# alipbcs/ZetaRay

Hardware: NVIDIA H100
Metric: Mpaths/s (1spp ReSTIR PT, 1080p) (higher is better)
Workload: dtype f32

## Files before the change

### zetaray_b200/csrc/rdi.cu

```cuda
#include "zr_pixel.cuh"
#include "zr_planes.h"
#include "zr_schedule.h"

#include "zr_rdi.cuh"

namespace zr
{
namespace
{
#ifndef ZR_RDI_THREADS
#define ZR_RDI_THREADS 512
#endif
    template<uint32_t MF>
    __global__ void ZR_LB(ZR_RDI_THREADS) k_di_temporal(SceneDev sc, FrameView f, DIParams prm, zr_rdi_reservoir* __restrict__ resCurr,
        const zr_rdi_reservoir* __restrict__ resPrev, uint2* __restrict__ target, float4* __restrict__ finalImg, uint32_t dispX, uint32_t dispY,
        const uint32_t* __restrict__ order)
    {
        using SD = BSDF::ShadingDataT<MF>;
        const zr_frame_constants& fc = f.fc;
        uint2 sg = make_uint2(0, 0);
        const uint32_t groupFlat = order[blockIdx.x] * (ZR_RDI_THREADS / 64) + (threadIdx.x >> 6);
        const uint32_t tInGroup = threadIdx.x & 63;
        uint2 px = make_uint2(0xffffffffu, 0xffffffffu);
        if (groupFlat < dispX * dispY)
            px = SwizzleThreadGroup(groupFlat, 0, tInGroup & 7, tInGroup >> 3, 8, 8, dispX, 16, 4, 16 * dispY, sg);
        const long long t0 = clock64();
        bool act = !(px.x >= f.W || px.y >= f.H || px.y < prm.rowBegin || px.y >= prm.rowEnd);
        const uint32_t x = px.x, y = px.y;
        const size_t idx = act ? (size_t)y * f.W + x : 0;
        if (act)
        {
            const GFlags flags = FlagsAt(f.core, f.W, x, y);
            if (flags.invalid)
            {
                finalImg[idx] = f4(0, 0, 0, 0);
                act = false;
// ... 5 lines not shown
            }
        }
        PixelT<SD> p;
        p.surface = SD::InitEmpty();
        p.pos = f3(0); p.normal = f3(0); p.roughness = 0;
        RNG rng_thread; rng_thread.State = 0;
        int numBsdfSamples = 0;
        if (act)
        {
            p = LoadPixel<SD>(f, sc, f.core, f.coat, x, y, false, x, y);
            rng_thread = RNG::Init(x, y, fc.FrameNum);
            numBsdfSamples = (!p.surface.GlossSpecular() && p.roughness < 0.3f) ? 2 : 1;
        }
        RNG rng_group = RNG::Init(groupFlat % dispX, groupFlat / dispX, fc.FrameNum);
        const uint32_t sampleSetIdx = rng_group.UniformUintBounded_Faster(sc.numSampleSets);
        Reservoir r = RIS_InitialCandidates_Sync(act, sc, p.pos, p.normal, p.roughness, p.surface, sampleSetIdx, numBsdfSamples, rng_thread);
        if (prm.temporal)
        {
            float2 motionVec = f2(0, 0);
            TemporalCandidateT<SD> tc; tc.valid = false; tc.px = tc.py = 0; tc.pos = tc.normal = f3(0);
            tc.surface = SD::InitEmpty();
            ZR_PHASE();
            if (act)
            {
                motionVec = unpack_snorm16x2(__ldg(&f.me[idx].x));
                const float2 currUV = f2((float)x + 0.5f, (float)y + 0.5f) / f2((float)f.W, (float)f.H);
                const float2 prevUV = currUV - motionVec;
                tc = FindTemporalCandidate(f, sc, p.pos, p.normal, p.roughness, p.surface, prevUV);
            }
            TemporalResample1_Sync(act && tc.valid, sc, p.pos, p.normal, p.surface, tc, resPrev, f.W, r, rng_thread);
            if (act && prm.spatial)
// ... 6 lines not shown
        }
        AccountCost(prm.costMap, f.W, f.H, px.x, px.y, t0);
        if (!act)
            return;
        if (prm.temporal || prm.reset)
        {
            zr_rdi_reservoir rec;
            r.Write(rec, prm.M_max);
            StoreRdi(&resCurr[idx], rec);
        }
        if (!prm.spatial || !prm.temporal)
            WriteFinal(fc, finalImg, idx, r.target * r.W);
    }

    template<uint32_t MF>
    __global__ void ZR_LB(ZR_RDI_THREADS) k_di_spatial(SceneDev sc, FrameView f, DIParams prm, const zr_rdi_reservoir* __restrict__ resCurr,
        const uint2* __restrict__ target, float4* __restrict__ finalImg, uint32_t dispX, uint32_t dispY,
        const uint32_t* __restrict__ order)
    {
        using SD = BSDF::ShadingDataT<MF>;
        const zr_frame_constants& fc = f.fc;
        uint2 sg = make_uint2(0, 0);
        const uint32_t groupFlat = order[blockIdx.x] * (ZR_RDI_THREADS / 64) + (threadIdx.x >> 6);
        const uint32_t tInGroup = threadIdx.x & 63;
        uint2 px = make_uint2(0xffffffffu, 0xffffffffu);
        if (groupFlat < dispX * dispY)
            px = SwizzleThreadGroup(groupFlat, 0, tInGroup & 7, tInGroup >> 3, 8, 8, dispX, 16, 4, 16 * dispY, sg);
        const long long t0 = clock64();
        bool active = px.x < f.W && px.y < f.H && px.y >= prm.rowBegin && px.y < prm.rowEnd;
        const int x = (int)px.x, y = (int)px.y;
        const size_t idx = active ? (size_t)y * f.W + x : 0;
        if (active)
        {
            const GFlags flags = FlagsAt(f.core, f.W, x, y);
            if (flags.invalid) active = false;
            else if (flags.emissive)
            {
                WriteEmissive(fc, f, finalImg, idx);
// ... 115 lines not shown
    } sz;
    int currTemporalIdx = 0;
    bool isTemporalReservoirValid = false;
    bool resetTemporalTextures = true;
    bool patternLoaded = false;
    zr_direct_params params = Defaults();
    zr::LightingStrip strip{ "zr_direct_pass" };

    static zr_direct_params Defaults()
    {
        zr_direct_params p{};
        p.temporal_resample = 1; p.spatial_resample = 1; p.stochastic_spatial = 1; p.extra_disocclusion_sampling = 1;
        p.M_max = 20; p.alpha_min = 0.05f * 0.05f;
        return p;
    }
    zr_status Setup() { return ZR_OK; }
    zr_status OnWindowResized(uint32_t w, uint32_t h)
    {
        const size_t n = (size_t)w * h;
        Sized next;
        for (int i = 0; i < 2; i++) ZR_TRY(next.planes.Alloc(next.d_res[i], n));
        ZR_TRY(next.planes.Alloc(next.d_target, n));
        ZR_TRY(next.planes.Alloc(next.d_final, n));
        ZR_TRY(next.planes.Clear());
        sz = std::move(next);
        width = w; height = h;
        strip.ForgetSize();
        ResetFlags();
        return ZR_OK;
    }
    void ResetFlags() { currTemporalIdx = 0; isTemporalReservoirValid = false; resetTemporalTextures = true; }
// ... 20 lines not shown
        zr_status st = LightingFrame("zr_direct_pass", in, width, height, f);
        if (st != ZR_OK) return st;
        st = LoadPattern();
        if (st != ZR_OK) return st;
        const bool doTemporal = isTemporalReservoirValid && params.temporal_resample;
        const bool doSpatial = doTemporal && params.spatial_resample;
        if (doTemporal && (!in->prev.d_core || !in->prev.d_coat))
        {
            set_error("zr_direct_pass_render: temporal reuse needs the previous G-buffer");
            return ZR_ERR_INVALID_ARG;
        }
        DIParams prm{ doTemporal, doSpatial, params.stochastic_spatial, params.extra_disocclusion_sampling, params.M_max,
            params.alpha_min, resetTemporalTextures, strip.rowBegin, strip.ClampedRowEnd(height), strip.d_costMap };
        const uint32_t dispX = (width + 7) / 8, dispY = (height + 7) / 8;
        const int cur = currTemporalIdx;
        st = strip.Schedule(width, height, 8, 8, ZR_RDI_THREADS / 64);
        if (st != ZR_OK) return st;
        const BlockSchedule& sched = strip.sched;
        const bool plain = (in->scene->materialFeatures & BSDF::MF_ALL) == 0;
        ZR_PROF("k_di_temporal", stream);
        (plain ? k_di_temporal<BSDF::MF_NONE> : k_di_temporal<BSDF::MF_ALL>)<<<sched.count, ZR_RDI_THREADS, 0, stream>>>(in->scene->dev, f, prm, sz.d_res[cur], sz.d_res[1 - cur], sz.d_target, sz.d_final, dispX, dispY, sched.d_order);
        ZR_LAUNCH_CHECK();
        strip.Exchange(sz.d_res[cur], width, height, 32u, stream);
        if (doSpatial)
        {
            ZR_PROF("k_di_spatial", stream);
            (plain ? k_di_spatial<BSDF::MF_NONE> : k_di_spatial<BSDF::MF_ALL>)<<<sched.count, ZR_RDI_THREADS, 0, stream>>>(in->scene->dev, f, prm, sz.d_res[cur], sz.d_target, sz.d_final, dispX, dispY, sched.d_order);
            ZR_LAUNCH_CHECK();
        }
        isTemporalReservoirValid = true;
        currTemporalIdx = 1 - cur;
        resetTemporalTextures = false;
        return ZR_OK;
    }
};

extern "C"
{
    zr_status zr_direct_pass_create(uint32_t width, uint32_t height, zr_direct_pass** out) { return zr::CreatePass("zr_direct_pass", width, height, out); }
    zr_status zr_direct_pass_resize(zr_direct_pass* p, uint32_t width, uint32_t height) { return zr::ResizePass("zr_direct_pass", p, width, height); }
    zr_status zr_direct_pass_reset_temporal(zr_direct_pass* p) { return zr::ResetPass(p); }
    zr_status zr_direct_pass_default_params(zr_direct_params* out) { return zr::DefaultParams<zr_direct_pass>(out); }
// ... 46 lines not shown
```

### zetaray_b200/csrc/rgi.cu

```cuda
#define ZR_NO_DEGENERATE_RAY_EARLY_OUT
#include "zr_pixel.cuh"
#include "zr_rpt.cuh"
#include "zr_planes.h"
#include "zr_schedule.h"

#include "zr_rgi.cuh"

namespace zr
{
namespace
{
#ifndef ZR_RGI_THREADS
#define ZR_RGI_THREADS 1024
#endif
    template<bool PlainPT>
    __global__ void ZR_LB(ZR_RGI_THREADS) k_rgi(SceneDev sc, FrameView f, GIParams prm, zr_rgi_reservoir* __restrict__ resCurr,
        const zr_rgi_reservoir* __restrict__ resPrev, float4* __restrict__ finalImg, uint32_t dispX, uint32_t dispY,
        const uint32_t* __restrict__ order)
    {
        const zr_frame_constants& fc = f.fc;
        uint2 sg = make_uint2(0, 0);
        const uint32_t groupFlat = order[blockIdx.x] * (ZR_RGI_THREADS / 64) + (threadIdx.x >> 6);
        const uint32_t tInGroup = threadIdx.x & 63;
        uint2 px = make_uint2(0xffffffffu, 0xffffffffu);
// ... 278 lines not shown
        {
            set_error("zr_gi_pass_render: the light voxel grid is enabled but zr_build_light_voxel_grid has not run");
            return ZR_ERR_NOT_INITIALIZED;
        }
        const bool doTemporal = !plainPathTracer && params.temporal_resample && isTemporalReservoirValid;
        if (doTemporal && !in->prev.d_core)
        {
            set_error("zr_gi_pass_render: temporal reuse needs the previous G-buffer");
            return ZR_ERR_INVALID_ARG;
        }
        GIParams prm{ params.max_non_tr_bounces, params.max_glossy_tr_bounces, params.russian_roulette, params.stochastic_multi_bounce,
            params.boiling_suppression, params.M_max, doTemporal ? 1u : 0u, resetTemporalTextures ? 1u : 0u, strip.rowBegin, strip.ClampedRowEnd(height) };
        const uint32_t dispX = (width + 7) / 8, dispY = (height + 7) / 8;
        st = strip.Schedule(width, height, 8, 8, ZR_RGI_THREADS / 64);
        if (st != ZR_OK) return st;
        const BlockSchedule& sched = strip.sched;
        const int cur = currTemporalIdx;
        if (plainPathTracer)
        {
            ZR_PROF("k_pathtracer", stream);
            k_rgi<true><<<sched.count, ZR_RGI_THREADS, 0, stream>>>(in->scene->dev, f, prm, sz.d_res[cur], sz.d_res[1 - cur], sz.d_final, dispX, dispY, sched.d_order);
            ZR_LAUNCH_CHECK();
            return ZR_OK;
        }
        ZR_PROF("k_rgi", stream);
        k_rgi<false><<<sched.count, ZR_RGI_THREADS, 0, stream>>>(in->scene->dev, f, prm, sz.d_res[cur], sz.d_res[1 - cur], sz.d_final, dispX, dispY, sched.d_order);
        ZR_LAUNCH_CHECK();
        strip.Exchange(sz.d_res[cur], width, height, (uint32_t)sizeof(zr_rgi_reservoir), stream);
        isTemporalReservoirValid = true;
        currTemporalIdx = 1 - cur;
        resetTemporalTextures = false;
// ... 57 lines not shown
```

### zetaray_b200/csrc/rpt.cu

```cuda
#include "zr_rpt_io.cuh"
#include "zr_rpt_spatial.h"
#include "zr_schedule.h"

namespace zr
{
namespace
{
    using namespace RPT;

    __device__ __align__(8) float c_disk512[1024];

#ifndef ZR_PT_THREADS
#define ZR_PT_THREADS 768
#endif
    struct PtParked
    {
        Reservoir r;
        Reconnection rc;
        uint32_t pad;
    };
    static_assert(sizeof(PtParked) % 4 == 0 && (sizeof(PtParked) / 4) % 2 == 1, "PtParked must be an odd number of words");
    constexpr size_t PT_SMEM_BYTES = (size_t)ZR_PT_THREADS * sizeof(PtParked);

    template<uint32_t MF>
// ... 459 lines not shown
    zr_indirect_params params = Defaults();

    static zr_indirect_params Defaults()
    {
        zr_indirect_params p{};
        p.max_non_tr_bounces = 3; p.max_glossy_tr_bounces = 4; p.russian_roulette = 1; p.temporal_resample = 1;
        p.num_spatial_passes = 1; p.M_max_temporal = 10; p.M_max_spatial = 8; p.boiling_suppression = 1;
        p.sort_temporal = 1; p.sort_spatial = 1; p.alpha_min = 0.175f * 0.175f;
        return p;
    }

    zr_status Setup()
    {
        decltype(&zr::k_pathtrace<zr::BSDF::MF_ALL>) const kernels[2] = { zr::k_pathtrace<zr::BSDF::MF_NONE>, zr::k_pathtrace<zr::BSDF::MF_ALL> };
        for (const auto kernel : kernels)
        {
            ZR_CUDA(cudaFuncSetAttribute(kernel, cudaFuncAttributeMaxDynamicSharedMemorySize, (int)zr::PT_SMEM_BYTES));
            int ptBlocks = 0;
            ZR_CUDA(cudaOccupancyMaxActiveBlocksPerMultiprocessor(&ptBlocks, kernel, ZR_PT_THREADS, zr::PT_SMEM_BYTES));
            if (ptBlocks < 1)
            {
                zr::set_error("zr_indirect_pass: k_pathtrace (%d threads, %zu B shared) cannot be resident", ZR_PT_THREADS, zr::PT_SMEM_BYTES);
                return ZR_ERR_UNSUPPORTED;
            }
            const size_t ptSmem = (size_t)ptBlocks * (zr::PT_SMEM_BYTES + 1024);
            ZR_CUDA(cudaFuncSetAttribute(kernel, cudaFuncAttributePreferredSharedMemoryCarveout,
                (int)((ptSmem * 100 + 228 * 1024 - 1) / (228 * 1024))));
        }
        return shiftStreams.Init();
    }

    zr_status OnWindowResized(uint32_t w, uint32_t h)
    {
        const size_t n = (size_t)w * h;
        Sized next;
        for (int i = 0; i < 2; i++) ZR_TRY(next.planes.Alloc(next.d_res[i], n));
        ZR_TRY(next.planes.Alloc(next.d_threadMap, n));
        ZR_TRY(next.planes.Alloc(next.d_target, n));
        ZR_TRY(next.planes.Alloc(next.d_final, n));
        ZR_TRY(next.planes.Alloc(next.d_neighbor, n));
        ZR_TRY(next.queued.Build(w, h, next.d_res[0], next.d_res[1]));
        ZR_TRY(next.planes.Clear());
        sz = std::move(next);
// ... 41 lines not shown
        RptParams prm;
        prm.maxNonTrBounces = params.max_non_tr_bounces; prm.maxGlossyTrBounces = params.max_glossy_tr_bounces;
        prm.russianRoulette = params.russian_roulette; prm.M_max_temporal = params.M_max_temporal; prm.M_max_spatial = params.M_max_spatial;
        prm.boilingSuppression = params.boiling_suppression; prm.sortSpatial = params.sort_spatial; prm.alpha_min = params.alpha_min;
        prm.temporalResample = doTemporal; prm.resetTemporal = resetTemporalTextures; prm.spatialFlag = doSpatial;
        prm.rowBegin = strip.rowBegin; prm.rowEnd = strip.ClampedRowEnd(height);
        prm.costMap = strip.d_costMap;
        st = strip.Schedule(width, height, 16, 8, ZR_PT_THREADS / 128);
        if (st != ZR_OK) return st;
        const uint32_t rows = prm.rowEnd - prm.rowBegin;

        int cur = currTemporalIdx;
        const uint32_t dispX = (width + 15) / 16, dispY = (height + 7) / 8;
        const bool plain = (in->scene->materialFeatures & BSDF::MF_ALL) == 0;
        ZR_PROF("k_pathtrace", stream);
        (plain ? k_pathtrace<BSDF::MF_NONE> : k_pathtrace<BSDF::MF_ALL>)<<<strip.sched.count, ZR_PT_THREADS, PT_SMEM_BYTES, stream>>>(in->scene->dev, f, prm, sz.d_res[cur], sz.d_target, sz.d_final, dispX, dispY,
            strip.sched.d_order);
        ZR_LAUNCH_CHECK();
        if (doTemporal)
        {
            st = sz.queued.RunTemporal(shiftStreams, in->scene->dev, f, prm, sz.d_res[cur], sz.d_res[1 - cur], sz.d_target, sz.d_final, plain, stream);
            if (st != ZR_OK) return st;
        }
        strip.Exchange(sz.d_res[cur], width, height, 64u, stream);
        if (doSpatial)
        {
            for (uint32_t pass = 0; pass < params.num_spatial_passes; pass++)
            {
                ZR_PROF("k_spatial_search", stream);
                k_spatial_search<<<dim3((width + 31) / 32, (rows + 7) / 8), 256, 0, stream>>>(f, prm, sz.d_neighbor);
                ZR_LAUNCH_CHECK();
                zr_rpt_reservoir* rin = sz.d_res[cur];
// ... 82 lines not shown
```

### zetaray_b200/csrc/rpt_spatial.cu

```cuda
#include "zr_rpt_spatial.h"
#include "zr_rpt_shift.cuh"
#include "zr_tma.cuh"

namespace zr
{
namespace
{
    using namespace RPT;

    __global__ void __launch_bounds__(256) k_spatial_classify(FrameView f, RptParams prm, const zr_rpt_reservoir* __restrict__ resIn,
        const uint16_t* __restrict__ neighbor, uint32_t* __restrict__ queue, uint32_t* __restrict__ counters, uint32_t capacity)
    {
        __shared__ uint32_t s_count[SpatialQueued::NUM_CLASSES], s_base[SpatialQueued::NUM_CLASSES];
        const uint32_t x = blockIdx.x * 32 + (threadIdx.x & 31);
        const uint32_t y = prm.rowBegin + blockIdx.y * 8 + (threadIdx.x >> 5);
        if (threadIdx.x < SpatialQueued::NUM_CLASSES) s_count[threadIdx.x] = 0;
        __syncthreads();
        uint32_t cls[2] = { NO_ITEM, NO_ITEM };
        if (x < f.W && y < f.H && y < prm.rowEnd)
        {
            const GFlags flags = FlagsAt(f.core, f.W, (int)x, (int)y);
            int nx = 0, ny = 0;
            if (!(flags.invalid || flags.emissive) && NeighborOf(f, neighbor, (int)x, (int)y, nx, ny))
            {
// ... 252 lines not shown
                        CopyToNextFrame(rec, &resOut[idx], r_curr, M_max);
                    WriteOutputColor(fc, finalImg, idx, r_curr.target * r_curr.W);
                }
            }
            __syncthreads();
        }
    }
}

zr_status ShiftStreams::Init()
{
    int dev = 0;
    ZR_CUDA(cudaGetDevice(&dev));
    ZR_CUDA(cudaDeviceGetAttribute(&numSMs, cudaDevAttrMultiProcessorCount, dev));
    ZR_CUDA(cudaFuncSetAttribute(k_spatial_merge, cudaFuncAttributeMaxDynamicSharedMemorySize, (int)sizeof(MergeSmem)));
    for (int i = 0; i < 2; i++)
    {
        ZR_CUDA(cudaStreamCreateWithFlags(&aux[i], cudaStreamNonBlocking));
        ZR_CUDA(cudaEventCreateWithFlags(&evJoin[i], cudaEventDisableTiming));
    }
    ZR_CUDA(cudaEventCreateWithFlags(&evFork, cudaEventDisableTiming));
    return ZR_OK;
}

ShiftStreams::~ShiftStreams()
{
    for (int i = 0; i < 2; i++)
    {
        if (aux[i]) cudaStreamDestroy(aux[i]);
        if (evJoin[i]) cudaEventDestroy(evJoin[i]);
// ... 74 lines not shown
```

### zetaray_b200/csrc/rpt_temporal.cu

```cuda
#include "zr_rpt_spatial.h"
#include "zr_rpt_shift.cuh"

namespace zr
{
namespace
{
    using namespace RPT;
    enum : uint8_t { TF_OK = 1, TF_REPLAY_OK = 2 };

    __global__ void __launch_bounds__(256) k_temporal_classify(SceneDev sc, FrameView f, RptParams prm, const zr_rpt_reservoir* __restrict__ resCurr,
        const zr_rpt_reservoir* __restrict__ resPrev, uint8_t* __restrict__ tflags, uint32_t* __restrict__ queue, uint32_t* __restrict__ counters,
        uint32_t capacity)
    {
        __shared__ uint32_t s_count[SpatialQueued::NUM_CLASSES], s_base[SpatialQueued::NUM_CLASSES];
        const int x = (int)(blockIdx.x * 32 + (threadIdx.x & 31));
        const int y = (int)(prm.rowBegin + blockIdx.y * 8 + (threadIdx.x >> 5));
        if (threadIdx.x < SpatialQueued::NUM_CLASSES) s_count[threadIdx.x] = 0;
        __syncthreads();
        uint32_t cls[2] = { NO_ITEM, NO_ITEM };
        uint32_t flagBits = 0;
        if (x < (int)f.W && y < (int)f.H && y < (int)prm.rowEnd)
        {
            const size_t idx = (size_t)y * f.W + x;
            const GFlags flags = DecodeFlags(ld128(&f.core[idx]).w & 0xff);
// ... 132 lines not shown
            {
                r_curr.target = Math::Sanitize(r_curr.target);
                target[idx] = f4(r_curr.target.x, r_curr.target.y, r_curr.target.z, 0.0f);
            }
        }
        else
        {
            r_curr.WriteReservoirData(rec, M_max);
            st128(&resCurr[idx], make_uint4(rec.meta, asuint(rec.w_sum), asuint(rec.W), rec.L_b));
        }
        if (!prm.spatialFlag)
            WriteOutputColor(fc, finalImg, idx, r_curr.target * r_curr.W);
    }
}

zr_status SpatialQueued::RunTemporal(const ShiftStreams& ss, const SceneDev& sc, const FrameView& f, const RptParams& prm, zr_rpt_reservoir* resCurr,
    const zr_rpt_reservoir* resPrev, float4* target, float4* finalImg, bool plain, cudaStream_t stream)
{
    const uint32_t rows = prm.rowEnd - prm.rowBegin;
    const dim3 grid((width + 31) / 32, (rows + 7) / 8);
    ZR_CUDA(cudaMemsetAsync(d_counters, 0, 16 * sizeof(uint32_t), stream));
    {
        ZR_PROF("k_temporal_classify", stream);
        k_temporal_classify<<<grid, 256, 0, stream>>>(sc, f, prm, resCurr, resPrev, d_flags, d_queue, d_counters, (uint32_t)capacity);
        ZR_LAUNCH_CHECK();
    }
    {
        ZR_PROF("k_shift_temporal", stream);
        const zr_status ls = LaunchShifts<true>(*this, ss, sc, f, prm, resCurr, resPrev, nullptr, plain, stream);
        zr::prof_after();
// ... 13 lines not shown
```

### zetaray_b200/csrc/zr_common.cuh

```cuda
#pragma once
#include <cuda_runtime.h>
#include <stdint.h>
#include "../../include/zr_abi.h"
#include "../../include/zr_fpmath.h"

#define ZR_D __device__ __forceinline__
#ifndef ZR_MAXREGS
#define ZR_MAXREGS 0
#endif
#if ZR_MAXREGS > 0
#define ZR_LB(threads) __launch_bounds__(threads, 65536 / ((threads) * ZR_MAXREGS))
#else
#define ZR_LB(threads) __launch_bounds__(threads)
#endif

namespace zr
{
constexpr float PI = 3.141592654f;
constexpr float TWO_PI = 6.283185307f;
constexpr float PI_OVER_2 = 1.570796327f;
constexpr float PI_OVER_4 = 0.7853981635f;
constexpr float ONE_OVER_PI = 0.318309886f;
constexpr float ONE_OVER_2_PI = 0.159154943f;
constexpr float FLT_MAX_ = 3.402823466e+38f;
constexpr float FLT16_MAX = 65504.0f;

void set_error(const char* fmt, ...);
zr_status read_asset(const char* who, const char* name, void* dst, size_t bytes);
zr_status cuda_fail(cudaError_t e, const char* what);
zr_status check_frame_size(const char* pass, const zr_frame_constants& frame, uint32_t width, uint32_t height);
void count_launch(uint64_t n = 1);
#define ZR_CUDA(expr) do { cudaError_t e__ = (expr); if (e__ != cudaSuccess) return zr::cuda_fail(e__, #expr); } while (0)
#define ZR_CLEAR_BEGIN() ZR_CUDA(cudaDeviceSynchronize())
#define ZR_CLEAR_END() ZR_CUDA(cudaStreamSynchronize(cudaStreamLegacy))
void prof_before(const char* name, cudaStream_t stream);
void prof_after();
#define ZR_PROF(name, stream) zr::prof_before(name, (cudaStream_t)(stream))
#define ZR_LAUNCH_CHECK() do { zr::count_launch(); zr::prof_after(); cudaError_t e__ = cudaGetLastError(); if (e__ != cudaSuccess) return zr::cuda_fail(e__, "kernel launch"); } while (0)

ZR_D float3 f3(float x, float y, float z) { return make_float3(x, y, z); }
ZR_D float3 f3(float s) { return make_float3(s, s, s); }
ZR_D float2 f2(float x, float y) { return make_float2(x, y); }
ZR_D float4 f4(float x, float y, float z, float w) { return make_float4(x, y, z, w); }

ZR_D float3 operator+(float3 a, float3 b) { return f3(a.x + b.x, a.y + b.y, a.z + b.z); }
ZR_D float3 operator-(float3 a, float3 b) { return f3(a.x - b.x, a.y - b.y, a.z - b.z); }
ZR_D float3 operator*(float3 a, float3 b) { return f3(a.x * b.x, a.y * b.y, a.z * b.z); }
ZR_D float3 operator/(float3 a, float3 b) { return f3(a.x / b.x, a.y / b.y, a.z / b.z); }
ZR_D float3 operator*(float3 a, float s) { return f3(a.x * s, a.y * s, a.z * s); }
// ... 447 lines not shown
```

### zetaray_b200/csrc/zr_rdi.cuh

```cuda
#pragma once
#include "zr_pixel.cuh"

namespace zr
{
namespace
{
    struct DIParams
    {
        uint32_t temporal, spatial, stochasticSpatial, extraDisocclusion, M_max; float alpha_min; uint32_t reset;
        uint32_t rowBegin, rowEnd;
        unsigned long long* costMap;
    };

    __constant__ float c_disk32[64];

struct Reservoir
{
    float w_sum, W; float3 le; uint32_t lightIdx; float2 bary; uint32_t M;
    float3 target; uint32_t lightID; float3 lightPos, lightNormal; bool doubleSided;

    static ZR_D Reservoir Init()
    {
        Reservoir r;
        r.le = f3(0); r.M = 0; r.w_sum = 0; r.W = 0; r.lightIdx = UINT32_MAX_; r.bary = f2(0, 0);
// ... 99 lines not shown
    {
        wi = lightPos - pos;
        t = dot(wi, wi) == 0 ? 0 : length(wi);
        wi = t == 0 ? f3(0) : wi / t;
        lightNormal = doubleSided && dot(-wi, lightNormal) < 0 ? -lightNormal : lightNormal;
    }
    ZR_D float dWdA() const
    {
        float cosThetaPrime = saturate(dot(lightNormal, -wi));
        return t == 0 ? 0 : cosThetaPrime / (t * t);
    }
};

#define ZR_PHASE() __syncthreads()
template<class SD>
ZR_D Reservoir RIS_InitialCandidates_Sync(bool act, const SceneDev& sc, float3 pos, float3 normal, float roughness, SD surface,
    uint32_t sampleSetIdx, int numBsdfSamples, RNG& rng)
{
    Reservoir r = Reservoir::Init();
    const bool specular = surface.GlossSpecular() && (surface.metallic || surface.specTr) && (!surface.Coated() || surface.CoatSpecular());
    const int numLightSamples = !specular ? 3 : 0;
    for (int s_b = 0; s_b < 2; s_b++)
    {
        const bool go = act && (s_b < numBsdfSamples);
        BSDF::BSDFSample bsdfSample = BSDF::BSDFSample::Init();
        ZR_PHASE();
        if (go)
            bsdfSample = BSDF::SampleBSDF_NoDiffuse(normal, surface, rng);
        ZR_PHASE();
        BSDFHitInfo hitInfo;
        hitInfo.hit = false;
        if (go)
            hitInfo = FindClosestHitDI(sc, pos, normal, bsdfSample.wi, surface.Transmissive());
        ZR_PHASE();
// ... 70 lines not shown
            target *= Visibility_Segment(sc, pos, wi, t, normal, lightID, surface.Transmissive()) ? 1.0f : 0.0f;
        ZR_PHASE();
        if (go)
        {
            const float denom = (float)numLightSamples * pdf_light + (float)numBsdfSamples * BSDF::BSDFSamplerPdf_NoDiffuse(normal, surface, wi) * dwdA;
            const float m_l = denom > 0 ? 1.0f / denom : 0;
            const float w_l = m_l * Math::Luminance(target);
            if (r.Update(w_l, le, emissiveIdx, lightSample.bary, rng))
            {
                r.target = target; r.lightID = lightID; r.lightNormal = lightSample.normal; r.lightPos = lightSample.pos; r.doubleSided = doubleSided;
            }
        }
    }
    float targetLum = Math::Luminance(r.target);
    r.W = targetLum > 0.0f ? r.w_sum / targetLum : 0.0f;
    return r;
}

ZR_D bool PlaneHeuristicDI(float3 samplePos, float3 currNormal, float3 currPos, float linearDepth, float tolerance = 1e-1f)
{
    float planeDist = dot(currNormal, samplePos - currPos);
    return fabsf(planeDist) <= tolerance * linearDepth;
}

template<class SD>
struct TemporalCandidateT { SD surface; float3 pos, normal; int px, py; bool valid; };
using TemporalCandidate = TemporalCandidateT<BSDF::ShadingData>;

template<class SD>
ZR_D TemporalCandidateT<SD> FindTemporalCandidate(const FrameView& f, const SceneDev& sc, float3 pos, float3 normal, float roughness, const SD& surface, float2 prevUV)
// ... 241 lines not shown
```

### zetaray_b200/csrc/zr_rpt_shift.cuh

```cuda
#pragma once
#include "zr_rpt_spatial.h"

namespace zr
{
namespace
{
    using namespace RPT;
#ifndef ZR_SHIFT_THREADS
#define ZR_SHIFT_THREADS 512
#endif
#ifndef ZR_SHIFT_MINBLOCKS
#define ZR_SHIFT_MINBLOCKS 1
#endif
    constexpr int SHIFT_THREADS = ZR_SHIFT_THREADS, SHIFT_MINBLOCKS = ZR_SHIFT_MINBLOCKS;
    constexpr uint32_t NO_ITEM = 0xffffffffu;

    ZR_D uint32_t ShiftClass(uint32_t meta)
    {
        const uint32_t kMin2 = meta & 0xf;
        const uint32_t lt_k = (meta >> 14) & 3, lt_k1 = (meta >> 16) & 3;
        const uint32_t c = lt_k1 != 0 ? 1u : (lt_k != 0 ? 2u : 0u);
        return c * 2 + (kMin2 > 0 ? 1u : 0u);
    }


    template<int CASE, bool REPLAY, bool TEMPORAL, uint32_t MF>
    __global__ void __launch_bounds__(SHIFT_THREADS, SHIFT_MINBLOCKS) k_shift(SceneDev sc, FrameView f, RptParams prm,
        const zr_rpt_reservoir* __restrict__ resIn, const zr_rpt_reservoir* __restrict__ resPrev, const uint16_t* __restrict__ neighbor,
        const uint32_t* __restrict__ queue, uint32_t* __restrict__ counters, uint32_t cls, ShiftResult* __restrict__ out)
    {
        using SD = BSDF::ShadingDataT<MF>;
        __shared__ uint32_t s_base;
        const uint32_t total = counters[cls];
        for (;;)
        {
            __syncthreads();
            if (threadIdx.x == 0) s_base = atomicAdd(&counters[8 + cls], (uint32_t)SHIFT_THREADS);
            __syncthreads();
            const uint32_t base = s_base;
            if (base >= total) break;
            const bool act = base + threadIdx.x < total;
            int x = 0, y = 0;
            uint32_t dir = 0;
            bool replayOk = act;
            Reservoir r = Reservoir::Init();
            PixelT<SD> p, pr;
            if (act)
            {
                const uint32_t item = __ldg(&queue[base + threadIdx.x]);
                x = (int)(item & 0xffff); y = (int)((item >> 16) & 0x3fff); dir = item >> 31;
                zr_rpt_reservoir rec;
                if (!TEMPORAL)
                {
                    int nx = 0, ny = 0;
                    NeighborOf(f, neighbor, x, y, nx, ny);
                    LoadRecord(dir == 0 ? &resIn[(size_t)y * f.W + x] : &resIn[(size_t)ny * f.W + nx], rec);
                    r = Reservoir::Load_NonReconnection(rec);
                    r.rc.x_k_in_motion = false;
                    r.Load_Reconnection(rec);
                    if (dir == 0) p = LoadPixel<SD>(f, sc, f.core, f.coat, nx, ny, false, x, y);
                    else p = LoadPixel<SD>(f, sc, f.core, f.coat, x, y, false, x, y);
                    if (REPLAY)
                    {
                        if (dir == 0) pr = LoadPixel<SD>(f, sc, f.core, f.coat, nx, ny, false, nx, ny);
                        else pr = p;
                    }
                }
                else
                {
                    replayOk = ((item >> 30) & 1) != 0;
                    int ppx = 0, ppy = 0;
                    PrevPixel(f, x, y, ppx, ppy);
                    LoadRecord(dir == 0 ? &resIn[(size_t)y * f.W + x] : &resPrev[(size_t)ppy * f.W + ppx], rec);
                    r = Reservoir::Load_NonReconnection(rec);
                    r.Load_Reconnection(rec);
                    if (r.rc.IsCase1() || r.rc.IsCase2())
                    {
                        if (dir == 0) XkToPrev(sc, r.rc);
                        else XkToCurr(sc, r.rc);
                    }
                    if (dir == 0) p = LoadPixel<SD>(f, sc, f.pcore, f.pcoat, ppx, ppy, true, x, y);
                    else p = LoadPixel<SD>(f, sc, f.core, f.coat, x, y, false, x, y);
                    if (REPLAY) pr = p;
                }
            }
            OffsetPathContextT<SD> ctx = OffsetPathContextT<SD>::Init();
            if (REPLAY)
            {
                ZR_PHASE();
                ctx = Replay_kGt2_Sync(act && replayOk, sc, pr.pos, pr.normal, pr.eta_next, pr.surface, r.rc, prm.alpha_min);
                if (act && replayOk)
                    ctx = ctx.Quantize();
            }
            const OffsetPath shift = Shift2_Sync<CASE>(act, sc, p.pos, p.normal, p.eta_next, p.surface, r.rc, &ctx, prm.alpha_min);
            if (act)
            {
                ShiftResult* o = &out[(size_t)y * f.W + x];
                if (dir == 0)
                    *reinterpret_cast<float2*>(&o->ctsTargetLum) = f2(Math::Luminance(shift.target), shift.partialJacobian);
                else if (TEMPORAL)
                    st128(o, make_uint4(asuint(shift.target.x), asuint(shift.target.y), asuint(shift.target.z), asuint(shift.partialJacobian)));
                else
                {
                    const float J = shift.partialJacobian;
                    const float Jenc = J > 0 ? (shift.surfKMin1Tramsmissive ? -J : J) : 0.0f;
                    st128(o, make_uint4(asuint(shift.target.x), asuint(shift.target.y), asuint(shift.target.z), asuint(Jenc)));
                }
            }
        }
    }

    template<bool TEMPORAL>
    zr_status LaunchShifts(const SpatialQueued& q, const ShiftStreams& ss, const SceneDev& sc, const FrameView& f, const RptParams& prm,
        const zr_rpt_reservoir* resIn, const zr_rpt_reservoir* resPrev, const uint16_t* neighbor, bool plain, cudaStream_t stream)
    {
        const uint32_t grid = (uint32_t)ss.numSMs * SHIFT_MINBLOCKS;
        cudaStream_t s1 = ss.aux[0], s2 = ss.aux[1];
        ZR_CUDA(cudaEventRecord(ss.evFork, stream));
        ZR_CUDA(cudaStreamWaitEvent(s1, ss.evFork, 0));
        ZR_CUDA(cudaStreamWaitEvent(s2, ss.evFork, 0));
#define ZR_LAUNCH_SHIFT(CASE, REPLAY, CLS, STREAM) \
        (plain ? k_shift<CASE, REPLAY, TEMPORAL, BSDF::MF_NONE> : k_shift<CASE, REPLAY, TEMPORAL, BSDF::MF_ALL>)<<<grid, SHIFT_THREADS, 0, STREAM>>>(sc, f, prm, resIn, resPrev, neighbor, q.d_queue + (size_t)(CLS) * q.capacity, \
            q.d_counters, CLS, q.d_shift); \
        zr::count_launch()
        ZR_LAUNCH_SHIFT(1, false, 0, stream);
        ZR_LAUNCH_SHIFT(2, false, 2, s1);
        ZR_LAUNCH_SHIFT(3, false, 4, s2);
        ZR_LAUNCH_SHIFT(1, true, 1, s1);
        ZR_LAUNCH_SHIFT(2, true, 3, s2);
        ZR_LAUNCH_SHIFT(3, true, 5, stream);
#undef ZR_LAUNCH_SHIFT
        ZR_CUDA(cudaEventRecord(ss.evJoin[0], s1));
        ZR_CUDA(cudaEventRecord(ss.evJoin[1], s2));
        ZR_CUDA(cudaStreamWaitEvent(stream, ss.evJoin[0], 0));
        ZR_CUDA(cudaStreamWaitEvent(stream, ss.evJoin[1], 0));
        return ZR_OK;
    }

    ZR_D void AppendItems(const uint32_t cls[2], const uint32_t item[2], uint32_t* __restrict__ queue, uint32_t* __restrict__ counters,
        uint32_t capacity, uint32_t* s_count, uint32_t* s_base)
    {
        const uint32_t lane = threadIdx.x & 31;
        uint32_t offs[2] = { 0, 0 };
        const uint32_t lt = (1u << lane) - 1;
#pragma unroll
        for (uint32_t c = 0; c < SpatialQueued::NUM_CLASSES; c++)
        {
            const uint32_t m0 = __ballot_sync(0xffffffffu, cls[0] == c), m1 = __ballot_sync(0xffffffffu, cls[1] == c);
            const uint32_t n0 = __popc(m0), n = n0 + __popc(m1);
            uint32_t base = 0;
// ... 17 lines not shown
```

### zetaray_b200/csrc/zr_rpt_spatial.h

```cpp
#pragma once
#include <cuda.h>
#include "zr_planes.h"
#include "zr_rpt_io.cuh"

namespace zr
{
struct ShiftResult
{
    float stcTarget[3];
    float stcJacobian;
    float ctsTargetLum;
    float ctsJacobian;
    uint32_t pad[2];
};
static_assert(sizeof(ShiftResult) == 32, "ShiftResult is two 128-bit words");

struct ShiftStreams
{
    int numSMs = 0;
    cudaStream_t aux[2] = { nullptr, nullptr };
    cudaEvent_t evFork = nullptr, evJoin[2] = { nullptr, nullptr };
    ShiftStreams() = default;
    ShiftStreams(const ShiftStreams&) = delete;
    ShiftStreams& operator=(const ShiftStreams&) = delete;
    ~ShiftStreams();
    zr_status Init();
};

struct SpatialQueued
{
    static constexpr int NUM_CLASSES = 6;
    Planes planes{ "zr_indirect_pass" };
    uint32_t width = 0, height = 0;
    uint32_t* d_queue = nullptr;
    uint32_t* d_counters = nullptr;
    ShiftResult* d_shift = nullptr;
    uint8_t* d_flags = nullptr;
    size_t capacity = 0;
    const void* mapBase[2] = { nullptr, nullptr };
    CUtensorMap* d_maps = nullptr;
    bool swizzled = false;

// ... 9 lines not shown
```

### zetaray_b200/csrc/zr_schedule.h

```cpp
#pragma once
#include <algorithm>
#include <cstdint>
#include <vector>
#include <cuda_runtime.h>
#include "zr_common.cuh"

namespace zr
{
struct BlockSchedule
{
    uint32_t* d_order = nullptr;
    uint32_t count = 0;
    uint32_t rowBegin = 0xffffffffu, rowEnd = 0, costVersion = 0xffffffffu;

    BlockSchedule() = default;
    BlockSchedule(const BlockSchedule&) = delete;
    BlockSchedule& operator=(const BlockSchedule&) = delete;
    ~BlockSchedule() { Release(); }
    void Release() { if (d_order) cudaFree(d_order); d_order = nullptr; count = 0; rowBegin = 0xffffffffu; }
    bool UpToDate(uint32_t y0, uint32_t y1, uint32_t version) const { return d_order && rowBegin == y0 && rowEnd == y1 && costVersion == version; }
    cudaError_t Upload(const std::vector<uint32_t>& order, uint32_t y0, uint32_t y1, uint32_t version)
    {
        if (d_order) cudaFree(d_order);
        d_order = nullptr;
// ... 97 lines not shown
    void Exchange(const zr_image2d* planes, int n, cudaStream_t stream) const
    {
        if (exchange) exchange(exchangeUser, planes, n, stream);
    }
    void Exchange(void* d_plane, uint32_t width, uint32_t height, uint32_t texelBytes, cudaStream_t stream) const
    {
        const zr_image2d plane{ d_plane, width, height, width * texelBytes, texelBytes };
        Exchange(&plane, 1, stream);
    }
};

struct LightingStrip : StripRows
{
    unsigned long long* d_costMap = nullptr;
    TileCosts tileCosts;
    BlockSchedule sched;

    explicit LightingStrip(const char* passName) : StripRows(passName) {}
    void ForgetSize()
    {
        ForgetRows();
        d_costMap = nullptr;
        tileCosts = TileCosts{};
        sched.Release();
    }
    zr_status SetCostMap(void* d_cycles)
    {
        d_costMap = (unsigned long long*)d_cycles;
        return ZR_OK;
    }
    zr_status SetScheduleCosts(const double* h_tile_cost, uint32_t tiles_x, uint32_t tiles_y, uint32_t width, uint32_t height)
    {
        if (h_tile_cost && (tiles_x != (width + 31) / 32 || tiles_y != (height + 31) / 32))
        {
            set_error("%s_set_schedule_costs: expected %u x %u tiles", pass, (width + 31) / 32, (height + 31) / 32);
            return ZR_ERR_INVALID_ARG;
        }
        tileCosts.cost.assign(h_tile_cost ? h_tile_cost : nullptr, h_tile_cost ? h_tile_cost + (size_t)tiles_x * tiles_y : nullptr);
        tileCosts.tilesX = h_tile_cost ? tiles_x : 0;
        tileCosts.version++;
        return ZR_OK;
    }
    zr_status Schedule(uint32_t width, uint32_t height, uint32_t groupW, uint32_t groupH, uint32_t groupsPerBlock)
    {
        const uint32_t y0 = rowBegin, y1 = ClampedRowEnd(height), v = tileCosts.version;
        if (!sched.UpToDate(y0, y1, v))
            ZR_CUDA(sched.Upload(ScheduleSwizzled((width + groupW - 1) / groupW, (height + groupH - 1) / groupH, groupW, groupH, groupsPerBlock,
                y0, y1, tileCosts), y0, y1, v));
        return ZR_OK;
    }
};
}
```

Baseline: 313.4.

## Park DI and shift reservoirs in shared memory and raise block sizes to 768

The DI temporal kernel now keeps its Reservoir in a padded per-thread dynamic shared-memory slot, and the shift kernels do the same for their Reconnection. This takes those values out of registers so blocks of 768 threads can fit, up from 512. A shared helper sets the dynamic-smem limit and the shared-memory carveout for these kernels and for the path tracer, and the lighting strip now keeps a separate block schedule per block shape. The trade-off is extra shared-memory traffic and a smaller L1 share in exchange for more resident warps.

```diff
diff --git a/zetaray_b200/csrc/rdi.cu b/zetaray_b200/csrc/rdi.cu
--- a/zetaray_b200/csrc/rdi.cu
+++ b/zetaray_b200/csrc/rdi.cu
@@ -8,18 +8,31 @@
 {
 namespace
 {
-#ifndef ZR_RDI_THREADS
-#define ZR_RDI_THREADS 512
+#ifndef ZR_RDI_TEMPORAL_THREADS
+#define ZR_RDI_TEMPORAL_THREADS 768
 #endif
+#ifndef ZR_RDI_SPATIAL_THREADS
+#define ZR_RDI_SPATIAL_THREADS 512
+#endif
+    static_assert(ZR_RDI_TEMPORAL_THREADS % 64 == 0 && ZR_RDI_SPATIAL_THREADS % 64 == 0, "a DI block is whole 8x8 groups");
+    struct DiTemporalParked
+    {
+        Reservoir r;
+        uint32_t pad[2];
+    };
+    static_assert(sizeof(DiTemporalParked) % 16 == 8, "DiTemporalParked must be 2 mod 4 words");
+    constexpr size_t DI_TEMPORAL_SMEM_BYTES = (size_t)ZR_RDI_TEMPORAL_THREADS * sizeof(DiTemporalParked);
+
     template<uint32_t MF>
-    __global__ void ZR_LB(ZR_RDI_THREADS) k_di_temporal(SceneDev sc, FrameView f, DIParams prm, zr_rdi_reservoir* __restrict__ resCurr,
+    __global__ void ZR_LB(ZR_RDI_TEMPORAL_THREADS) k_di_temporal(SceneDev sc, FrameView f, DIParams prm, zr_rdi_reservoir* __restrict__ resCurr,
         const zr_rdi_reservoir* __restrict__ resPrev, uint2* __restrict__ target, float4* __restrict__ finalImg, uint32_t dispX, uint32_t dispY,
         const uint32_t* __restrict__ order)
     {
         using SD = BSDF::ShadingDataT<MF>;
+        extern __shared__ DiTemporalParked s_diTemporalParked[];
         const zr_frame_constants& fc = f.fc;
         uint2 sg = make_uint2(0, 0);
-        const uint32_t groupFlat = order[blockIdx.x] * (ZR_RDI_THREADS / 64) + (threadIdx.x >> 6);
+        const uint32_t groupFlat = order[blockIdx.x] * (ZR_RDI_TEMPORAL_THREADS / 64) + (threadIdx.x >> 6);
         const uint32_t tInGroup = threadIdx.x & 63;
         uint2 px = make_uint2(0xffffffffu, 0xffffffffu);
         if (groupFlat < dispX * dispY)
@@ -55,7 +68,8 @@
         }
         RNG rng_group = RNG::Init(groupFlat % dispX, groupFlat / dispX, fc.FrameNum);
         const uint32_t sampleSetIdx = rng_group.UniformUintBounded_Faster(sc.numSampleSets);
-        Reservoir r = RIS_InitialCandidates_Sync(act, sc, p.pos, p.normal, p.roughness, p.surface, sampleSetIdx, numBsdfSamples, rng_thread);
+        Reservoir& r = s_diTemporalParked[threadIdx.x].r;
+        RIS_InitialCandidates_Sync(r, act, sc, p.pos, p.normal, p.roughness, p.surface, sampleSetIdx, numBsdfSamples, rng_thread);
         if (prm.temporal)
         {
             float2 motionVec = f2(0, 0);
@@ -92,14 +106,14 @@
     }
 
     template<uint32_t MF>
-    __global__ void ZR_LB(ZR_RDI_THREADS) k_di_spatial(SceneDev sc, FrameView f, DIParams prm, const zr_rdi_reservoir* __restrict__ resCurr,
+    __global__ void ZR_LB(ZR_RDI_SPATIAL_THREADS) k_di_spatial(SceneDev sc, FrameView f, DIParams prm, const zr_rdi_reservoir* __restrict__ resCurr,
         const uint2* __restrict__ target, float4* __restrict__ finalImg, uint32_t dispX, uint32_t dispY,
         const uint32_t* __restrict__ order)
     {
         using SD = BSDF::ShadingDataT<MF>;
         const zr_frame_constants& fc = f.fc;
         uint2 sg = make_uint2(0, 0);
-        const uint32_t groupFlat = order[blockIdx.x] * (ZR_RDI_THREADS / 64) + (threadIdx.x >> 6);
+        const uint32_t groupFlat = order[blockIdx.x] * (ZR_RDI_SPATIAL_THREADS / 64) + (threadIdx.x >> 6);
         const uint32_t tInGroup = threadIdx.x & 63;
         uint2 px = make_uint2(0xffffffffu, 0xffffffffu);
         if (groupFlat < dispX * dispY)
@@ -245,7 +259,13 @@
         p.M_max = 20; p.alpha_min = 0.05f * 0.05f;
         return p;
     }
-    zr_status Setup() { return ZR_OK; }
+    zr_status Setup()
+    {
+        using zr::BSDF::MF_NONE; using zr::BSDF::MF_ALL;
+        ZR_TRY(zr::ReserveParkedSmem(zr::k_di_temporal<MF_NONE>, ZR_RDI_TEMPORAL_THREADS, zr::DI_TEMPORAL_SMEM_BYTES, "zr_direct_pass: k_di_temporal"));
+        ZR_TRY(zr::ReserveParkedSmem(zr::k_di_temporal<MF_ALL>, ZR_RDI_TEMPORAL_THREADS, zr::DI_TEMPORAL_SMEM_BYTES, "zr_direct_pass: k_di_temporal"));
+        return ZR_OK;
+    }
     zr_status OnWindowResized(uint32_t w, uint32_t h)
     {
         const size_t n = (size_t)w * h;
@@ -296,18 +316,21 @@
             params.alpha_min, resetTemporalTextures, strip.rowBegin, strip.ClampedRowEnd(height), strip.d_costMap };
         const uint32_t dispX = (width + 7) / 8, dispY = (height + 7) / 8;
         const int cur = currTemporalIdx;
-        st = strip.Schedule(width, height, 8, 8, ZR_RDI_THREADS / 64);
-        if (st != ZR_OK) return st;
-        const BlockSchedule& sched = strip.sched;
+        st = strip.Schedule(width, height, 8, 8, ZR_RDI_TEMPORAL_THREADS / 64, 0);
+        if (st != ZR_OK) return st;
+        st = strip.Schedule(width, height, 8, 8, ZR_RDI_SPATIAL_THREADS / 64, 1);
+        if (st != ZR_OK) return st;
+        const BlockSchedule& schedT = strip.sched[0];
+        const BlockSchedule& schedS = strip.sched[1];
         const bool plain = (in->scene->materialFeatures & BSDF::MF_ALL) == 0;
         ZR_PROF("k_di_temporal", stream);
-        (plain ? k_di_temporal<BSDF::MF_NONE> : k_di_temporal<BSDF::MF_ALL>)<<<sched.count, ZR_RDI_THREADS, 0, stream>>>(in->scene->dev, f, prm, sz.d_res[cur], sz.d_res[1 - cur], sz.d_target, sz.d_final, dispX, dispY, sched.d_order);
+        (plain ? k_di_temporal<BSDF::MF_NONE> : k_di_temporal<BSDF::MF_ALL>)<<<schedT.count, ZR_RDI_TEMPORAL_THREADS, DI_TEMPORAL_SMEM_BYTES, stream>>>(in->scene->dev, f, prm, sz.d_res[cur], sz.d_res[1 - cur], sz.d_target, sz.d_final, dispX, dispY, schedT.d_order);
         ZR_LAUNCH_CHECK();
         strip.Exchange(sz.d_res[cur], width, height, 32u, stream);
         if (doSpatial)
         {
             ZR_PROF("k_di_spatial", stream);
-            (plain ? k_di_spatial<BSDF::MF_NONE> : k_di_spatial<BSDF::MF_ALL>)<<<sched.count, ZR_RDI_THREADS, 0, stream>>>(in->scene->dev, f, prm, sz.d_res[cur], sz.d_target, sz.d_final, dispX, dispY, sched.d_order);
+            (plain ? k_di_spatial<BSDF::MF_NONE> : k_di_spatial<BSDF::MF_ALL>)<<<schedS.count, ZR_RDI_SPATIAL_THREADS, 0, stream>>>(in->scene->dev, f, prm, sz.d_res[cur], sz.d_target, sz.d_final, dispX, dispY, schedS.d_order);
             ZR_LAUNCH_CHECK();
         }
         isTemporalReservoirValid = true;
diff --git a/zetaray_b200/csrc/rgi.cu b/zetaray_b200/csrc/rgi.cu
--- a/zetaray_b200/csrc/rgi.cu
+++ b/zetaray_b200/csrc/rgi.cu
@@ -316,7 +316,7 @@
         const uint32_t dispX = (width + 7) / 8, dispY = (height + 7) / 8;
         st = strip.Schedule(width, height, 8, 8, ZR_RGI_THREADS / 64);
         if (st != ZR_OK) return st;
-        const BlockSchedule& sched = strip.sched;
+        const BlockSchedule& sched = strip.sched[0];
         const int cur = currTemporalIdx;
         if (plainPathTracer)
         {
diff --git a/zetaray_b200/csrc/rpt.cu b/zetaray_b200/csrc/rpt.cu
--- a/zetaray_b200/csrc/rpt.cu
+++ b/zetaray_b200/csrc/rpt.cu
@@ -497,19 +497,7 @@
     {
         decltype(&zr::k_pathtrace<zr::BSDF::MF_ALL>) const kernels[2] = { zr::k_pathtrace<zr::BSDF::MF_NONE>, zr::k_pathtrace<zr::BSDF::MF_ALL> };
         for (const auto kernel : kernels)
-        {
-            ZR_CUDA(cudaFuncSetAttribute(kernel, cudaFuncAttributeMaxDynamicSharedMemorySize, (int)zr::PT_SMEM_BYTES));
-            int ptBlocks = 0;
-            ZR_CUDA(cudaOccupancyMaxActiveBlocksPerMultiprocessor(&ptBlocks, kernel, ZR_PT_THREADS, zr::PT_SMEM_BYTES));
-            if (ptBlocks < 1)
-            {
-                zr::set_error("zr_indirect_pass: k_pathtrace (%d threads, %zu B shared) cannot be resident", ZR_PT_THREADS, zr::PT_SMEM_BYTES);
-                return ZR_ERR_UNSUPPORTED;
-            }
-            const size_t ptSmem = (size_t)ptBlocks * (zr::PT_SMEM_BYTES + 1024);
-            ZR_CUDA(cudaFuncSetAttribute(kernel, cudaFuncAttributePreferredSharedMemoryCarveout,
-                (int)((ptSmem * 100 + 228 * 1024 - 1) / (228 * 1024))));
-        }
+            ZR_TRY(zr::ReserveParkedSmem(kernel, ZR_PT_THREADS, zr::PT_SMEM_BYTES, "zr_indirect_pass: k_pathtrace"));
         return shiftStreams.Init();
     }
 
@@ -581,8 +569,8 @@
         const uint32_t dispX = (width + 15) / 16, dispY = (height + 7) / 8;
         const bool plain = (in->scene->materialFeatures & BSDF::MF_ALL) == 0;
         ZR_PROF("k_pathtrace", stream);
-        (plain ? k_pathtrace<BSDF::MF_NONE> : k_pathtrace<BSDF::MF_ALL>)<<<strip.sched.count, ZR_PT_THREADS, PT_SMEM_BYTES, stream>>>(in->scene->dev, f, prm, sz.d_res[cur], sz.d_target, sz.d_final, dispX, dispY,
-            strip.sched.d_order);
+        (plain ? k_pathtrace<BSDF::MF_NONE> : k_pathtrace<BSDF::MF_ALL>)<<<strip.sched[0].count, ZR_PT_THREADS, PT_SMEM_BYTES, stream>>>(in->scene->dev, f, prm, sz.d_res[cur], sz.d_target, sz.d_final, dispX, dispY,
+            strip.sched[0].d_order);
         ZR_LAUNCH_CHECK();
         if (doTemporal)
         {
diff --git a/zetaray_b200/csrc/rpt_spatial.cu b/zetaray_b200/csrc/rpt_spatial.cu
--- a/zetaray_b200/csrc/rpt_spatial.cu
+++ b/zetaray_b200/csrc/rpt_spatial.cu
@@ -290,6 +290,8 @@
     ZR_CUDA(cudaGetDevice(&dev));
     ZR_CUDA(cudaDeviceGetAttribute(&numSMs, cudaDevAttrMultiProcessorCount, dev));
     ZR_CUDA(cudaFuncSetAttribute(k_spatial_merge, cudaFuncAttributeMaxDynamicSharedMemorySize, (int)sizeof(MergeSmem)));
+    ZR_TRY(SetupShifts<false>());
+    ZR_TRY(SetupTemporalShifts());
     for (int i = 0; i < 2; i++)
     {
         ZR_CUDA(cudaStreamCreateWithFlags(&aux[i], cudaStreamNonBlocking));
diff --git a/zetaray_b200/csrc/rpt_temporal.cu b/zetaray_b200/csrc/rpt_temporal.cu
--- a/zetaray_b200/csrc/rpt_temporal.cu
+++ b/zetaray_b200/csrc/rpt_temporal.cu
@@ -170,6 +170,11 @@
     }
 }
 
+zr_status SetupTemporalShifts()
+{
+    return SetupShifts<true>();
+}
+
 zr_status SpatialQueued::RunTemporal(const ShiftStreams& ss, const SceneDev& sc, const FrameView& f, const RptParams& prm, zr_rpt_reservoir* resCurr,
     const zr_rpt_reservoir* resPrev, float4* target, float4* finalImg, bool plain, cudaStream_t stream)
 {
diff --git a/zetaray_b200/csrc/zr_common.cuh b/zetaray_b200/csrc/zr_common.cuh
--- a/zetaray_b200/csrc/zr_common.cuh
+++ b/zetaray_b200/csrc/zr_common.cuh
@@ -33,6 +33,21 @@
 #define ZR_CUDA(expr) do { cudaError_t e__ = (expr); if (e__ != cudaSuccess) return zr::cuda_fail(e__, #expr); } while (0)
 #define ZR_CLEAR_BEGIN() ZR_CUDA(cudaDeviceSynchronize())
 #define ZR_CLEAR_END() ZR_CUDA(cudaStreamSynchronize(cudaStreamLegacy))
+template<class Kernel>
+zr_status ReserveParkedSmem(Kernel kernel, int threads, size_t bytes, const char* what)
+{
+    ZR_CUDA(cudaFuncSetAttribute(kernel, cudaFuncAttributeMaxDynamicSharedMemorySize, (int)bytes));
+    int blocks = 0;
+    ZR_CUDA(cudaOccupancyMaxActiveBlocksPerMultiprocessor(&blocks, kernel, threads, bytes));
+    if (blocks < 1)
+    {
+        set_error("%s (%d threads, %zu B shared) cannot be resident", what, threads, bytes);
+        return ZR_ERR_UNSUPPORTED;
+    }
+    const size_t smem = (size_t)blocks * (bytes + 1024);
+    ZR_CUDA(cudaFuncSetAttribute(kernel, cudaFuncAttributePreferredSharedMemoryCarveout, (int)((smem * 100 + 228 * 1024 - 1) / (228 * 1024))));
+    return ZR_OK;
+}
 void prof_before(const char* name, cudaStream_t stream);
 void prof_after();
 #define ZR_PROF(name, stream) zr::prof_before(name, (cudaStream_t)(stream))
diff --git a/zetaray_b200/csrc/zr_rdi.cuh b/zetaray_b200/csrc/zr_rdi.cuh
--- a/zetaray_b200/csrc/zr_rdi.cuh
+++ b/zetaray_b200/csrc/zr_rdi.cuh
@@ -137,10 +137,10 @@
 
 #define ZR_PHASE() __syncthreads()
 template<class SD>
-ZR_D Reservoir RIS_InitialCandidates_Sync(bool act, const SceneDev& sc, float3 pos, float3 normal, float roughness, SD surface,
+ZR_D void RIS_InitialCandidates_Sync(Reservoir& r, bool act, const SceneDev& sc, float3 pos, float3 normal, float roughness, SD surface,
     uint32_t sampleSetIdx, int numBsdfSamples, RNG& rng)
 {
-    Reservoir r = Reservoir::Init();
+    r = Reservoir::Init();
     const bool specular = surface.GlossSpecular() && (surface.metallic || surface.specTr) && (!surface.Coated() || surface.CoatSpecular());
     const int numLightSamples = !specular ? 3 : 0;
     for (int s_b = 0; s_b < 2; s_b++)
@@ -241,6 +241,13 @@
     }
     float targetLum = Math::Luminance(r.target);
     r.W = targetLum > 0.0f ? r.w_sum / targetLum : 0.0f;
+}
+template<class SD>
+ZR_D Reservoir RIS_InitialCandidates_Sync(bool act, const SceneDev& sc, float3 pos, float3 normal, float roughness, SD surface,
+    uint32_t sampleSetIdx, int numBsdfSamples, RNG& rng)
+{
+    Reservoir r;
+    RIS_InitialCandidates_Sync(r, act, sc, pos, normal, roughness, surface, sampleSetIdx, numBsdfSamples, rng);
     return r;
 }
 
diff --git a/zetaray_b200/csrc/zr_rpt_shift.cuh b/zetaray_b200/csrc/zr_rpt_shift.cuh
--- a/zetaray_b200/csrc/zr_rpt_shift.cuh
+++ b/zetaray_b200/csrc/zr_rpt_shift.cuh
@@ -7,13 +7,21 @@
 {
     using namespace RPT;
 #ifndef ZR_SHIFT_THREADS
-#define ZR_SHIFT_THREADS 512
+#define ZR_SHIFT_THREADS 768
 #endif
 #ifndef ZR_SHIFT_MINBLOCKS
 #define ZR_SHIFT_MINBLOCKS 1
 #endif
     constexpr int SHIFT_THREADS = ZR_SHIFT_THREADS, SHIFT_MINBLOCKS = ZR_SHIFT_MINBLOCKS;
     constexpr uint32_t NO_ITEM = 0xffffffffu;
+
+    struct ShiftParked
+    {
+        Reconnection rc;
+        uint32_t pad;
+    };
+    static_assert(sizeof(ShiftParked) % 4 == 0 && (sizeof(ShiftParked) / 4) % 2 == 1, "ShiftParked must be an odd number of words");
+    constexpr size_t SHIFT_SMEM_BYTES = (size_t)SHIFT_THREADS * sizeof(ShiftParked);
 
     ZR_D uint32_t ShiftClass(uint32_t meta)
     {
@@ -31,6 +39,8 @@
     {
         using SD = BSDF::ShadingDataT<MF>;
         __shared__ uint32_t s_base;
+        extern __shared__ ShiftParked s_shiftParked[];
+        Reconnection& rc = s_shiftParked[threadIdx.x].rc;
         const uint32_t total = counters[cls];
         for (;;)
         {
@@ -43,7 +53,6 @@
             int x = 0, y = 0;
             uint32_t dir = 0;
             bool replayOk = act;
-            Reservoir r = Reservoir::Init();
             PixelT<SD> p, pr;
             if (act)
             {
@@ -55,9 +64,10 @@
                     int nx = 0, ny = 0;
                     NeighborOf(f, neighbor, x, y, nx, ny);
                     LoadRecord(dir == 0 ? &resIn[(size_t)y * f.W + x] : &resIn[(size_t)ny * f.W + nx], rec);
-                    r = Reservoir::Load_NonReconnection(rec);
+                    Reservoir r = Reservoir::Load_NonReconnection(rec);
                     r.rc.x_k_in_motion = false;
                     r.Load_Reconnection(rec);
+                    rc = r.rc;
                     if (dir == 0) p = LoadPixel<SD>(f, sc, f.core, f.coat, nx, ny, false, x, y);
                     else p = LoadPixel<SD>(f, sc, f.core, f.coat, x, y, false, x, y);
                     if (REPLAY)
@@ -72,27 +82,30 @@
                     int ppx = 0, ppy = 0;
                     PrevPixel(f, x, y, ppx, ppy);
                     LoadRecord(dir == 0 ? &resIn[(size_t)y * f.W + x] : &resPrev[(size_t)ppy * f.W + ppx], rec);
-                    r = Reservoir::Load_NonReconnection(rec);
+                    Reservoir r = Reservoir::Load_NonReconnection(rec);
                     r.Load_Reconnection(rec);
                     if (r.rc.IsCase1() || r.rc.IsCase2())
                     {
                         if (dir == 0) XkToPrev(sc, r.rc);
                         else XkToCurr(sc, r.rc);
                     }
+                    rc = r.rc;
                     if (dir == 0) p = LoadPixel<SD>(f, sc, f.pcore, f.pcoat, ppx, ppy, true, x, y);
                     else p = LoadPixel<SD>(f, sc, f.core, f.coat, x, y, false, x, y);
                     if (REPLAY) pr = p;
                 }
             }
+            else
+                rc = Reconnection::Init();
             OffsetPathContextT<SD> ctx = OffsetPathContextT<SD>::Init();
             if (REPLAY)
             {
                 ZR_PHASE();
-                ctx = Replay_kGt2_Sync(act && replayOk, sc, pr.pos, pr.normal, pr.eta_next, pr.surface, r.rc, prm.alpha_min);
+                ctx = Replay_kGt2_Sync(act && replayOk, sc, pr.pos, pr.normal, pr.eta_next, pr.surface, rc, prm.alpha_min);
                 if (act && replayOk)
                     ctx = ctx.Quantize();
             }
-            const OffsetPath shift = Shift2_Sync<CASE>(act, sc, p.pos, p.normal, p.eta_next, p.surface, r.rc, &ctx, prm.alpha_min);
+            const OffsetPath shift = Shift2_Sync<CASE>(act, sc, p.pos, p.normal, p.eta_next, p.surface, rc, &ctx, prm.alpha_min);
             if (act)
             {
                 ShiftResult* o = &out[(size_t)y * f.W + x];
@@ -120,7 +133,7 @@
         ZR_CUDA(cudaStreamWaitEvent(s1, ss.evFork, 0));
         ZR_CUDA(cudaStreamWaitEvent(s2, ss.evFork, 0));
 #define ZR_LAUNCH_SHIFT(CASE, REPLAY, CLS, STREAM) \
-        (plain ? k_shift<CASE, REPLAY, TEMPORAL, BSDF::MF_NONE> : k_shift<CASE, REPLAY, TEMPORAL, BSDF::MF_ALL>)<<<grid, SHIFT_THREADS, 0, STREAM>>>(sc, f, prm, resIn, resPrev, neighbor, q.d_queue + (size_t)(CLS) * q.capacity, \
+        (plain ? k_shift<CASE, REPLAY, TEMPORAL, BSDF::MF_NONE> : k_shift<CASE, REPLAY, TEMPORAL, BSDF::MF_ALL>)<<<grid, SHIFT_THREADS, SHIFT_SMEM_BYTES, STREAM>>>(sc, f, prm, resIn, resPrev, neighbor, q.d_queue + (size_t)(CLS) * q.capacity, \
             q.d_counters, CLS, q.d_shift); \
         zr::count_launch()
         ZR_LAUNCH_SHIFT(1, false, 0, stream);
@@ -134,6 +147,20 @@
         ZR_CUDA(cudaEventRecord(ss.evJoin[1], s2));
         ZR_CUDA(cudaStreamWaitEvent(stream, ss.evJoin[0], 0));
         ZR_CUDA(cudaStreamWaitEvent(stream, ss.evJoin[1], 0));
+        return ZR_OK;
+    }
+
+    template<bool TEMPORAL>
+    zr_status SetupShifts()
+    {
+        using BSDF::MF_NONE; using BSDF::MF_ALL;
+        decltype(&k_shift<1, false, TEMPORAL, MF_ALL>) const kernels[12] = {
+            k_shift<1, false, TEMPORAL, MF_NONE>, k_shift<2, false, TEMPORAL, MF_NONE>, k_shift<3, false, TEMPORAL, MF_NONE>,
+            k_shift<1, true, TEMPORAL, MF_NONE>, k_shift<2, true, TEMPORAL, MF_NONE>, k_shift<3, true, TEMPORAL, MF_NONE>,
+            k_shift<1, false, TEMPORAL, MF_ALL>, k_shift<2, false, TEMPORAL, MF_ALL>, k_shift<3, false, TEMPORAL, MF_ALL>,
+            k_shift<1, true, TEMPORAL, MF_ALL>, k_shift<2, true, TEMPORAL, MF_ALL>, k_shift<3, true, TEMPORAL, MF_ALL> };
+        for (const auto kernel : kernels)
+            ZR_TRY(ReserveParkedSmem(kernel, SHIFT_THREADS, SHIFT_SMEM_BYTES, "zr_indirect_pass: k_shift"));
         return ZR_OK;
     }
 
diff --git a/zetaray_b200/csrc/zr_rpt_spatial.h b/zetaray_b200/csrc/zr_rpt_spatial.h
--- a/zetaray_b200/csrc/zr_rpt_spatial.h
+++ b/zetaray_b200/csrc/zr_rpt_spatial.h
@@ -26,6 +26,7 @@
     ~ShiftStreams();
     zr_status Init();
 };
+zr_status SetupTemporalShifts();
 
 struct SpatialQueued
 {
diff --git a/zetaray_b200/csrc/zr_schedule.h b/zetaray_b200/csrc/zr_schedule.h
--- a/zetaray_b200/csrc/zr_schedule.h
+++ b/zetaray_b200/csrc/zr_schedule.h
@@ -135,7 +135,7 @@
 {
     unsigned long long* d_costMap = nullptr;
     TileCosts tileCosts;
-    BlockSchedule sched;
+    BlockSchedule sched[2];
 
     explicit LightingStrip(const char* passName) : StripRows(passName) {}
     void ForgetSize()
@@ -143,7 +143,8 @@
         ForgetRows();
         d_costMap = nullptr;
         tileCosts = TileCosts{};
-        sched.Release();
+        sched[0].Release();
+        sched[1].Release();
     }
     zr_status SetCostMap(void* d_cycles)
     {
@@ -162,11 +163,12 @@
         tileCosts.version++;
         return ZR_OK;
     }
-    zr_status Schedule(uint32_t width, uint32_t height, uint32_t groupW, uint32_t groupH, uint32_t groupsPerBlock)
+    zr_status Schedule(uint32_t width, uint32_t height, uint32_t groupW, uint32_t groupH, uint32_t groupsPerBlock, int shape = 0)
     {
         const uint32_t y0 = rowBegin, y1 = ClampedRowEnd(height), v = tileCosts.version;
-        if (!sched.UpToDate(y0, y1, v))
-            ZR_CUDA(sched.Upload(ScheduleSwizzled((width + groupW - 1) / groupW, (height + groupH - 1) / groupH, groupW, groupH, groupsPerBlock,
+        BlockSchedule& s = sched[shape];
+        if (!s.UpToDate(y0, y1, v))
+            ZR_CUDA(s.Upload(ScheduleSwizzled((width + groupW - 1) / groupW, (height + groupH - 1) / groupH, groupW, groupH, groupsPerBlock,
                 y0, y1, tileCosts), y0, y1, v));
         return ZR_OK;
     }
```

New measurement: 323.9 (median of 6 runs). 1.03x the previous value.
